# ORNL/HydraGNN

Measured on NVIDIA H100. Metric: atoms_per_sec_training_step, higher is better.
Workload: dtype tf32

## Files before the change

### hydragnn_b200/csrc/hgb_tc.cu

```cuda
#include "hgb_tc.cuh"

namespace {

__device__ __forceinline__ void wgmma_n32(float* d, uint64_t ad, uint64_t bd) {
  asm volatile(
      "{\n"
      ".reg .pred p;\n"
      "setp.ne.b32 p, %18, 0;\n"
      "wgmma.mma_async.sync.aligned.m64n32k8.f32.tf32.tf32 "
      "{%0, %1, %2, %3, %4, %5, %6, %7, %8, %9, %10, %11, %12, %13, %14, %15}, %16, %17, p, 1, 1;\n"
      "}"
      : "+f"(d[0]), "+f"(d[1]), "+f"(d[2]), "+f"(d[3]), "+f"(d[4]), "+f"(d[5]), "+f"(d[6]), "+f"(d[7]), "+f"(d[8]), "+f"(d[9]),
        "+f"(d[10]), "+f"(d[11]), "+f"(d[12]), "+f"(d[13]), "+f"(d[14]), "+f"(d[15])
      : "l"(ad), "l"(bd), "r"(1));
}
__device__ __forceinline__ void wgmma_n16(float* d, uint64_t ad, uint64_t bd) {
  asm volatile(
      "{\n"
      ".reg .pred p;\n"
      "setp.ne.b32 p, %10, 0;\n"
      "wgmma.mma_async.sync.aligned.m64n16k8.f32.tf32.tf32 "
      "{%0, %1, %2, %3, %4, %5, %6, %7}, %8, %9, p, 1, 1;\n"
      "}"
      : "+f"(d[0]), "+f"(d[1]), "+f"(d[2]), "+f"(d[3]), "+f"(d[4]), "+f"(d[5]), "+f"(d[6]), "+f"(d[7])
      : "l"(ad), "l"(bd), "r"(1));
}

__device__ __forceinline__ float tf32_rna(float x) { return __uint_as_float((__float_as_uint(x) + 0x1000u) & 0xffffe000u); }

__device__ __forceinline__ void split_f4(const float4 v, float4& h, float4& l) {
  h.x = tf32_rna(v.x); h.y = tf32_rna(v.y); h.z = tf32_rna(v.z); h.w = tf32_rna(v.w);
  l.x = tf32_rna(v.x - h.x); l.y = tf32_rna(v.y - h.y); l.z = tf32_rna(v.z - h.z); l.w = tf32_rna(v.w - h.w);
}

struct LinParams {
  int m, kr, no;
  const float* w;
  int64_t ldw;
  int trans_b;
  const float* bias;
  int act;
  float act_param;
  float* y;
  float* z;
  const float* addend;
  int64_t ldy;
  const float* gsrc;
  int gact;
  int z_deriv;
  int stages;
  int split;
  int slots;
};

struct LinParamsGA : LinParams {
  const float* gadd;
  const int32_t* gptr;
  int ng;
  int64_t ldg;
};
template <bool GA> struct LinParamsOf { using type = LinParams; };
template <> struct LinParamsOf<true> { using type = LinParamsGA; };

constexpr int TILE_M = 64;
constexpr uint32_t A_STAGE = TILE_M * 128;
constexpr uint32_t SUB_BYTES = TILE_M * 128;
constexpr int LIN_THREADS = 384;

enum { EPI_NONE, EPI_RELU, EPI_SILU, EPI_SILU_ZD, EPI_TANH, EPI_OTHER };

template <int K, bool GA>
__device__ __forceinline__ float lin_epilogue1(const LinParams& p, float v, float& z, float a, float g) {
  z = v;
  if (K == EPI_RELU) v = isnan(v) ? v : fmaxf(v, 0.f);
  if (K == EPI_SILU) v = __fdividef(v, 1.f + __expf(-v));
  if (K == EPI_SILU_ZD) {
    const float s = __fdividef(1.f, 1.f + __expf(-v));
    v *= s;
    z = fmaf(v, 1.f - s, s);
  }
  if (K == EPI_TANH) v = tanhf(v);
  if (K == EPI_OTHER) v = hgb_act(v, p.act, p.act_param);
  if (GA || p.addend) v += a;
  if (p.gsrc) {
    if (p.gact == HGB_ACT_RELU_SELECT) v = hgb_relu_select(v, g);
    else v *= p.gact == HGB_ACT_DERIV ? g : hgb_act_grad(g, g, p.gact, p.act_param);
  }
  return v;
}

template <int K, bool GA>
__device__ __forceinline__ void lin_epilogue_sub(const LinParams& p, const float* sb, uint8_t* ys, uint8_t* zs, int tid, const float4* a,
                                                 const float4* g) {
#pragma unroll
  for (int j = 0; j < 4; ++j) {
    const int idx = j * 128 + tid, r = idx >> 3, q = idx & 7;
    const uint32_t off = (uint32_t)r * 128 + ((q ^ (r & 7)) << 4);
    float4 v = *reinterpret_cast<float4*>(ys + off), z;
    v.x = lin_epilogue1<K, GA>(p, v.x + sb[4 * q], z.x, a[j].x, g[j].x);
    v.y = lin_epilogue1<K, GA>(p, v.y + sb[4 * q + 1], z.y, a[j].y, g[j].y);
    v.z = lin_epilogue1<K, GA>(p, v.z + sb[4 * q + 2], z.z, a[j].z, g[j].z);
    v.w = lin_epilogue1<K, GA>(p, v.w + sb[4 * q + 3], z.w, a[j].w, g[j].w);
    *reinterpret_cast<float4*>(ys + off) = v;
    if (zs) *reinterpret_cast<float4*>(zs + off) = z;
  }
}

__device__ __forceinline__ int lin_graph_of(const LinParamsGA& p, int row) {
  int lo = 0, hi = p.ng;
  while (hi - lo > 1) {
    const int mid = (lo + hi) >> 1;
    if (__ldg(p.gptr + mid) <= row) lo = mid; else hi = mid;
  }
  return lo;
}

template <bool GA>
__device__ __forceinline__ void lin_load_operands(const typename LinParamsOf<GA>::type& p, int row0, int c, int tid, const int* gid, float4* a, float4* g) {
#pragma unroll
  for (int j = 0; j < 4; ++j) {
    const int idx = j * 128 + tid, row = row0 + (idx >> 3);
    const int64_t o = (int64_t)row * p.ldy + c * 32 + (idx & 7) * 4;
    const bool in = row < p.m;
    if (p.addend) a[j] = in ? __ldg(reinterpret_cast<const float4*>(p.addend + o)) : make_float4(0.f, 0.f, 0.f, 0.f);
    if constexpr (GA)
      a[j] = in ? __ldg(reinterpret_cast<const float4*>(p.gadd + (int64_t)gid[j] * p.ldg + c * 32 + (idx & 7) * 4))
                : make_float4(0.f, 0.f, 0.f, 0.f);
    if (p.gsrc) g[j] = in ? __ldg(reinterpret_cast<const float4*>(p.gsrc + o)) : make_float4(0.f, 0.f, 0.f, 0.f);
  }
}

template <int NC, bool SPLIT, bool GA>
__global__ void __launch_bounds__(LIN_THREADS, 1) tc_linear_kernel(const __grid_constant__ CUtensorMap tmap_a,
                                                                   const __grid_constant__ CUtensorMap tmap_y,
                                                                   const __grid_constant__ CUtensorMap tmap_z,
                                                                   const typename LinParamsOf<GA>::type p) {
  constexpr int NO = NC * 32;
  extern __shared__ uint8_t smem_raw[];
  uint8_t* smem = reinterpret_cast<uint8_t*>((reinterpret_cast<uintptr_t>(smem_raw) + 1023) & ~(uintptr_t)1023);
  const int KB = p.kr >> 5;
  const uint32_t b_pad = ((uint32_t)KB * NO * 128 + 1023) & ~1023u;
  uint8_t* sB = smem;
  uint8_t* sBlo = sB + b_pad;
  uint8_t* sOut = sB + (SPLIT ? 2 : 1) * (size_t)b_pad;
  uint8_t* sA = sOut + (size_t)2 * p.slots * SUB_BYTES;
  const int S = p.stages;
  const int SR = S >> 1;
  uint8_t* sAlo = sA + (size_t)S * A_STAGE;
  uint64_t* full = reinterpret_cast<uint64_t*>(sA + (size_t)(SPLIT ? 2 : 1) * S * A_STAGE);
  uint64_t* empty = full + S;
  uint64_t* full2 = empty + S;
  float* sbias = reinterpret_cast<float*>(full2 + S);

  const int warp = threadIdx.x >> 5, lane = threadIdx.x & 31;
  const int ntiles = (p.m + TILE_M - 1) / TILE_M;
  for (int i = threadIdx.x; i < NO; i += blockDim.x) sbias[i] = p.bias ? __ldg(p.bias + i) : 0.f;
  if (threadIdx.x == 0) {
    for (int s = 0; s < S; ++s) { mbar_init(full + s, 1); mbar_init(empty + s, 4); mbar_init(full2 + s, 3); }
    fence_barrier_init();
  }
  __syncthreads();

  if (warp < 4) {
    regs_dec<PRODUCER_REGS>();
    if (warp == 0) {
    if (lane == 0) {
      uint32_t li = 0;
      for (int t = blockIdx.x; t < ntiles; t += gridDim.x, ++li)
        for (int kb = 0; kb < KB; ++kb) {
          const uint32_t n = (li >> 1) * KB + kb;
          const int s = (li & 1) * SR + n % SR;
          mbar_wait(empty + s, ((n / SR) & 1) ^ 1);
          mbar_expect_tx(full + s, A_STAGE);
          tma_load_2d(sA + (size_t)s * A_STAGE, &tmap_a, full + s, kb * 32, t * TILE_M);
        }
    }
    } else {
    if (SPLIT) {
      const int tl = threadIdx.x - 32;
      uint32_t li = 0;
      for (int t = blockIdx.x; t < ntiles; t += gridDim.x, ++li)
        for (int kb = 0; kb < KB; ++kb) {
          const uint32_t n = (li >> 1) * KB + kb;
          const int s = (li & 1) * SR + n % SR;
          mbar_wait(full + s, (n / SR) & 1);
          float4* pa = reinterpret_cast<float4*>(sA + (size_t)s * A_STAGE);
          float4* pl = reinterpret_cast<float4*>(sAlo + (size_t)s * A_STAGE);
          for (int idx = tl; idx < (int)(A_STAGE / 16); idx += 96) {
            float4 h, l;
            split_f4(pa[idx], h, l);
            pa[idx] = h;
            pl[idx] = l;
          }
          fence_proxy_async();
          __syncwarp();
          if (lane == 0) mbar_arrive(full2 + s);
        }
    }
    }
  } else {
    regs_inc<CONSUMER_REGS>();
    {
      const int total = NO * p.kr;
      constexpr int SU = 8;
      for (int base = threadIdx.x - 128; base < total; base += 256 * SU) {
        float val[SU];
        uint32_t off[SU];
#pragma unroll
        for (int u = 0; u < SU; ++u) {
          const int i = base + u * 256;
          val[u] = 0.f;
          off[u] = 0xffffffffu;
          if (i < total) {
            if (!p.trans_b) {
              const int r = i / p.kr, c = i - r * p.kr;
              off[u] = kmajor_sw128_off(r, c, NO);
              val[u] = __ldg(p.w + (int64_t)r * p.ldw + c);
            } else {
              const int c = i / NO, r = i - c * NO;
              off[u] = kmajor_sw128_off(r, c, NO);
              val[u] = __ldg(p.w + (int64_t)c * p.ldw + r);
            }
          }
        }
#pragma unroll
        for (int u = 0; u < SU; ++u)
          if (off[u] != 0xffffffffu) {
            if (SPLIT) {
              const float hi = tf32_rna(val[u]);
              *reinterpret_cast<float*>(sB + off[u]) = hi;
              *reinterpret_cast<float*>(sBlo + off[u]) = tf32_rna(val[u] - hi);
            } else {
              *reinterpret_cast<float*>(sB + off[u]) = val[u];
            }
          }
      }
      fence_proxy_async();
    }
    named_bar_sync(1, 256);
    const int cw = (warp - 4) >> 2;
    const int wq = warp & 3;
    const int tid = threadIdx.x & 127;
    const uint32_t sA_addr = smem_u32(sA), sAlo_addr = smem_u32(sAlo), sB_addr = smem_u32(sB), sBlo_addr = smem_u32(sBlo);
    uint8_t* sOwn = sOut + (size_t)cw * p.slots * SUB_BYTES;
    const int per_sub = p.z ? 2 : 1;
    const int ahead = p.slots / per_sub - 1;
    const int kind = p.act == HGB_ACT_NONE ? EPI_NONE
                     : p.act == HGB_ACT_RELU ? EPI_RELU
                     : p.act == HGB_ACT_SILU ? (p.z && p.z_deriv ? EPI_SILU_ZD : EPI_SILU)
                     : p.act == HGB_ACT_TANH ? EPI_TANH
                                             : EPI_OTHER;
    const bool operands = GA || p.addend || p.gsrc;
    float acc[NC * 16];
    uint32_t sub = 0;
    int li = cw;
    for (int t = blockIdx.x + cw * gridDim.x; t < ntiles; t += 2 * gridDim.x, li += 2) {
      const int row0 = t * TILE_M;
      int gid[4] = {0, 0, 0, 0};
      if constexpr (GA) {
#pragma unroll
        for (int j = 0; j < 4; ++j) {
          const int row = row0 + ((j * 128 + tid) >> 3);
          if (row < p.m) gid[j] = lin_graph_of(p, row);
        }
      }
      float4 opa[4], opg[4];
#pragma unroll
      for (int j = 0; j < 4; ++j) opa[j] = opg[j] = make_float4(0.f, 0.f, 0.f, 0.f);
      constexpr bool early = NC < 8;
      if (early && operands) lin_load_operands<GA>(p, row0, 0, tid, gid, opa, opg);
#pragma unroll
      for (int j = 0; j < NC * 16; ++j) acc[j] = 0.f;
      const uint32_t n0 = (uint32_t)(li >> 1) * KB;
      for (int kb = 0; kb < KB; ++kb) {
        const uint32_t n = n0 + kb;
        const int s = cw * SR + n % SR;
        mbar_wait(SPLIT ? full2 + s : full + s, (n / SR) & 1);
        fence_regs<NC * 16>(acc);
        wgmma_fence();
#pragma unroll
        for (int k4 = 0; k4 < 4; ++k4) {
          const uint64_t ad = make_desc(sA_addr + s * A_STAGE + k4 * 32);
          const uint32_t boff = (uint32_t)kb * NO * 128 + k4 * 32;
          const uint64_t bd = make_desc(sB_addr + boff);
          if (SPLIT) {
            wgmma_tf32<NC>(acc, make_desc(sAlo_addr + s * A_STAGE + k4 * 32), bd);
            wgmma_tf32<NC>(acc, ad, make_desc(sBlo_addr + boff));
          }
          wgmma_tf32<NC>(acc, ad, bd);
        }
        wgmma_commit();
        fence_regs<NC * 16>(acc);
        if (kb > 0) {
          wgmma_wait<1>();
          if (lane == 0) mbar_arrive(empty + cw * SR + (n - 1) % SR);
        }
      }
      wgmma_wait<0>();
      fence_regs<NC * 16>(acc);
      if (lane == 0) mbar_arrive(empty + cw * SR + (n0 + KB - 1) % SR);
      if (!early && operands) lin_load_operands<GA>(p, row0, 0, tid, gid, opa, opg);
#pragma unroll 1
      for (int c = 0; c < NC; ++c, ++sub) {
        uint8_t* ys = sOwn + (size_t)((sub % (p.slots / per_sub)) * per_sub) * SUB_BYTES;
        uint8_t* zs = p.z ? ys + SUB_BYTES : nullptr;
        if (tid == 0) {
          if (ahead == 0) bulk_wait_read<0>(); else if (ahead == 1) bulk_wait_read<1>(); else bulk_wait_read<3>();
        }
        named_bar_sync(2 + cw, 128);
#pragma unroll
        for (int cc = 0; cc < NC; ++cc)
          if (cc == c) {
#pragma unroll
            for (int i = 0; i < 4; ++i)
#pragma unroll
              for (int h = 0; h < 2; ++h) {
                const int r = wq * 16 + (lane >> 2) + 8 * h, col = i * 8 + 2 * (lane & 3);
                *reinterpret_cast<float2*>(ys + kmajor_sw128_off(r, col, TILE_M)) =
                    make_float2(acc[16 * cc + 4 * i + 2 * h], acc[16 * cc + 4 * i + 2 * h + 1]);
              }
          }
        named_bar_sync(2 + cw, 128);
        const float* sb = sbias + c * 32;
        switch (kind) {
          case EPI_NONE: lin_epilogue_sub<EPI_NONE, GA>(p, sb, ys, zs, tid, opa, opg); break;
          case EPI_RELU: lin_epilogue_sub<EPI_RELU, GA>(p, sb, ys, zs, tid, opa, opg); break;
          case EPI_SILU: lin_epilogue_sub<EPI_SILU, GA>(p, sb, ys, zs, tid, opa, opg); break;
          case EPI_SILU_ZD: lin_epilogue_sub<EPI_SILU_ZD, GA>(p, sb, ys, zs, tid, opa, opg); break;
          case EPI_TANH: lin_epilogue_sub<EPI_TANH, GA>(p, sb, ys, zs, tid, opa, opg); break;
          default: lin_epilogue_sub<EPI_OTHER, GA>(p, sb, ys, zs, tid, opa, opg);
        }
        if (operands && c + 1 < NC) lin_load_operands<GA>(p, row0, c + 1, tid, gid, opa, opg);
        fence_proxy_async();
        named_bar_sync(2 + cw, 128);
        if (tid == 0) {
          tma_store_2d(&tmap_y, ys, c * 32, row0);
          if (zs) tma_store_2d(&tmap_z, zs, c * 32, row0);
          bulk_commit();
        }
      }
    }
    if (tid == 0) bulk_wait_all();
  }
}

struct WgParams {
  int m, no, ko;
  int chunks_per_cta;
  int stages;
  int tbufs;
  int split;
  int flush;
  float* part;
};

constexpr int WG_ROWS = 32;
constexpr int WG_NA = 128;
constexpr int WG_THREADS = 384;

template <int Q, bool SPLIT>
__global__ void __launch_bounds__(WG_THREADS, 1) tc_wgrad_kernel(const __grid_constant__ CUtensorMap tmap_dz,
                                                                 const __grid_constant__ CUtensorMap tmap_x, const WgParams p) {
  constexpr int KO = 32 * Q, NB = KO + 16;
  constexpr uint32_t SLAB = WG_ROWS * 128;
  constexpr uint32_t HI_BYTES = (uint32_t)(WG_NA + NB) * 128;
  extern __shared__ uint8_t smem_raw[];
  uint8_t* smem = reinterpret_cast<uint8_t*>((reinterpret_cast<uintptr_t>(smem_raw) + 1023) & ~(uintptr_t)1023);
  const int n0 = blockIdx.y * WG_NA;
  const int nrows = min(WG_NA, p.no - n0);
  const int nsl = nrows >> 5;
  const uint32_t raw_bytes = (uint32_t)(nsl + Q) * SLAB;
  const uint32_t tb_bytes = HI_BYTES * (SPLIT ? 2 : 1);
  const int S = p.stages, T = p.tbufs;
  uint8_t* tbuf = smem;
  uint8_t* raw = smem + (size_t)T * tb_bytes;
  uint64_t* full = reinterpret_cast<uint64_t*>(raw + (size_t)S * raw_bytes);
  uint64_t* empty = full + S;
  const int warp = threadIdx.x >> 5, lane = threadIdx.x & 31;

  const int total_chunks = (p.m + WG_ROWS - 1) / WG_ROWS;
  const int c_beg = blockIdx.x * p.chunks_per_cta;
  const int nchunks = max(0, min(total_chunks, c_beg + p.chunks_per_cta) - c_beg);

  if (threadIdx.x == 0) {
    for (int s = 0; s < S; ++s) { mbar_init(full + s, 1); mbar_init(empty + s, 8); }
    fence_barrier_init();
  }
  for (int i = threadIdx.x; i < (int)(T * tb_bytes / 4); i += blockDim.x) {
    const uint32_t o = (uint32_t)i * 4 % tb_bytes;
    const bool lo = o >= HI_BYTES;
    const int row = (int)((lo ? o - HI_BYTES : o) / 128);
    reinterpret_cast<float*>(tbuf)[i] = (!lo && row >= WG_NA + KO) ? 1.f : 0.f;
  }
  fence_proxy_async();
  __syncthreads();

  if (warp >= 8) {
    regs_dec<PRODUCER_REGS>();
    if (warp == 8 && lane == 0) {
      for (int c = 0; c < nchunks; ++c) {
        const int s = c % S;
        mbar_wait(empty + s, ((c / S) & 1) ^ 1);
        mbar_expect_tx(full + s, raw_bytes);
        uint8_t* st = raw + (size_t)s * raw_bytes;
        const int row0 = (c_beg + c) * WG_ROWS;
        for (int j = 0; j < nsl; ++j) tma_load_2d(st + (size_t)j * SLAB, &tmap_dz, full + s, n0 + j * 32, row0);
        for (int j = 0; j < Q; ++j) tma_load_2d(st + (size_t)(nsl + j) * SLAB, &tmap_x, full + s, j * 32, row0);
      }
    }
    return;
  }

  regs_inc<CONSUMER_REGS>();
  const int wg = warp >> 2, wq = warp & 3;
  const bool mma_on = wg * 64 < nrows;
  const int rows_t = nsl * 32 + KO;
  float acc[Q][16], accb[8];
#pragma unroll
  for (int c = 0; c < Q; ++c)
#pragma unroll
    for (int j = 0; j < 16; ++j) acc[c][j] = 0.f;
#pragma unroll
  for (int j = 0; j < 8; ++j) accb[j] = 0.f;
  bool first = true;
  float* part = p.part + (size_t)blockIdx.x * p.no * (p.ko + 1);

  auto flush = [&]() {
    if (mma_on) {
      const int rb = n0 + wg * 64 + wq * 16 + (lane >> 2);
#pragma unroll
      for (int h = 0; h < 2; ++h) {
        const int row = rb + 8 * h;
        if (row < n0 + nrows) {
          float* pr = part + (size_t)row * (KO + 1);
#pragma unroll
          for (int c = 0; c < Q; ++c)
#pragma unroll
            for (int i = 0; i < 4; ++i)
#pragma unroll
              for (int e = 0; e < 2; ++e) {
                const int col = c * 32 + i * 8 + 2 * (lane & 3) + e;
                const float v = acc[c][4 * i + 2 * h + e];
                pr[col] = first ? v : pr[col] + v;
              }
          if ((lane & 3) == 0) pr[KO] = first ? accb[2 * h] : pr[KO] + accb[2 * h];
        }
      }
    }
    first = false;
#pragma unroll
    for (int c = 0; c < Q; ++c)
#pragma unroll
      for (int j = 0; j < 16; ++j) acc[c][j] = 0.f;
#pragma unroll
    for (int j = 0; j < 8; ++j) accb[j] = 0.f;
  };

  for (int c = 0; c < nchunks; ++c) {
    const int s = c % S;
    uint8_t* tb = tbuf + (size_t)(c % T) * tb_bytes;
    const uint8_t* st = raw + (size_t)s * raw_bytes;
    mbar_wait(full + s, (c / S) & 1);
    for (int it = threadIdx.x; it < rows_t * 8; it += 256) {
      const int r = it % rows_t, m4 = it / rows_t;
      const int slab = r < nrows ? r >> 5 : nsl + ((r - nrows) >> 5);
      const float* src = reinterpret_cast<const float*>(st + (size_t)slab * SLAB) + (r & 31) + m4 * 4 * 32;
      const float4 v = make_float4(src[0], src[32], src[64], src[96]);
      const int orow = r < nrows ? r : WG_NA + (r - nrows);
      const uint32_t off = (uint32_t)orow * 128 + ((m4 ^ (orow & 7)) << 4);
      if (SPLIT) {
        float4 h, l;
        split_f4(v, h, l);
        *reinterpret_cast<float4*>(tb + off) = h;
        *reinterpret_cast<float4*>(tb + HI_BYTES + off) = l;
      } else {
        *reinterpret_cast<float4*>(tb + off) = v;
      }
    }
    fence_proxy_async();
    __syncwarp();
    if (lane == 0) mbar_arrive(empty + s);
    named_bar_sync(1, 256);
    if (mma_on) {
      const uint32_t ta = smem_u32(tb);
      fence_regs<Q * 16>(&acc[0][0]);
      fence_regs<8>(accb);
      wgmma_fence();
#pragma unroll
      for (int k4 = 0; k4 < 4; ++k4) {
        const uint32_t aoff = (uint32_t)(wg * 64) * 128 + k4 * 32;
        const uint64_t ad = make_desc(ta + aoff), adl = make_desc(ta + HI_BYTES + aoff);
#pragma unroll
        for (int j = 0; j < Q; ++j) {
          const uint32_t boff = (uint32_t)WG_NA * 128 + (uint32_t)j * 4096 + k4 * 32;
          const uint64_t bd = make_desc(ta + boff);
          if (SPLIT) {
            wgmma_n32(acc[j], adl, bd);
            wgmma_n32(acc[j], ad, make_desc(ta + HI_BYTES + boff));
          }
          wgmma_n32(acc[j], ad, bd);
        }
        const uint64_t bones = make_desc(ta + (uint32_t)(WG_NA + KO) * 128 + k4 * 32);
        if (SPLIT) wgmma_n16(accb, adl, bones);
        wgmma_n16(accb, ad, bones);
      }
      wgmma_commit();
      fence_regs<Q * 16>(&acc[0][0]);
      fence_regs<8>(accb);
    }
    if (T == 2) wgmma_wait<1>(); else wgmma_wait<0>();
    if (p.flush && (c + 1) % p.flush == 0 && c + 1 < nchunks) {
      wgmma_wait<0>();
      fence_regs<Q * 16>(&acc[0][0]);
      fence_regs<8>(accb);
      flush();
    }
    named_bar_sync(2, 256);
  }
  wgmma_wait<0>();
  fence_regs<Q * 16>(&acc[0][0]);
  fence_regs<8>(accb);
  flush();
}

__global__ void tc_wgrad_reduce_kernel(const float* __restrict__ part, int nparts, int no, int ko, float* __restrict__ dw,
                                       int64_t lddw, float* __restrict__ db, int accumulate) {
  __shared__ float red[8][33];
  const int w = ko + 1;
  const int cnt = no * w;
  const int i = blockIdx.x * 32 + threadIdx.x;
  float acc = 0.f;
  if (i < cnt) {
    float a0 = 0.f, a1 = 0.f, a2 = 0.f, a3 = 0.f;
    int b = threadIdx.y;
    for (; b + 24 < nparts; b += 32) {
      a0 += part[(size_t)b * cnt + i]; a1 += part[(size_t)(b + 8) * cnt + i];
      a2 += part[(size_t)(b + 16) * cnt + i]; a3 += part[(size_t)(b + 24) * cnt + i];
    }
    for (; b < nparts; b += 8) a0 += part[(size_t)b * cnt + i];
    acc = (a0 + a1) + (a2 + a3);
  }
  red[threadIdx.y][threadIdx.x] = acc;
  __syncthreads();
  if (threadIdx.y == 0 && i < cnt) {
    float t = 0.f;
#pragma unroll
    for (int w8 = 0; w8 < 8; ++w8) t += red[w8][threadIdx.x];
    const int r = i / w, c = i % w;
    if (c == ko) {
      if (db) db[r] = accumulate ? db[r] + t : t;
    } else {
      float* o = dw + (int64_t)r * lddw + c;
      *o = accumulate ? *o + t : t;
    }
  }
}

bool shape_ok(int kr, int no) { return kr >= 32 && kr <= 256 && kr % 32 == 0 && no >= 32 && no <= 256 && no % 32 == 0; }

template <int NC, bool SPLIT, bool GA>
void launch_linear_t(int grid, size_t smem, cudaStream_t st, const CUtensorMap* tm, const typename LinParamsOf<GA>::type& p) {
  static bool attr_set = false;
  if (!attr_set) {
    cudaFuncSetAttribute(tc_linear_kernel<NC, SPLIT, GA>, cudaFuncAttributeMaxDynamicSharedMemorySize, (int)SMEM_MAX);
    attr_set = true;
  }
  tc_linear_kernel<NC, SPLIT, GA><<<grid, LIN_THREADS, smem, st>>>(tm[0], tm[1], tm[2], p);
}
template <int NC>
void launch_linear(int grid, size_t smem, cudaStream_t st, const CUtensorMap* tm, const LinParamsGA& p) {
  if (p.gadd) {
    if (p.split) launch_linear_t<NC, true, true>(grid, smem, st, tm, p); else launch_linear_t<NC, false, true>(grid, smem, st, tm, p);
  } else {
    const LinParams& q = p;
    if (q.split) launch_linear_t<NC, true, false>(grid, smem, st, tm, q); else launch_linear_t<NC, false, false>(grid, smem, st, tm, q);
  }
}

template <int Q, bool SPLIT>
void launch_wgrad_t(dim3 grid, size_t smem, cudaStream_t st, const CUtensorMap& tdz, const CUtensorMap& tx, const WgParams& p) {
  static bool attr_set = false;
  if (!attr_set) {
    cudaFuncSetAttribute(tc_wgrad_kernel<Q, SPLIT>, cudaFuncAttributeMaxDynamicSharedMemorySize, (int)SMEM_MAX);
    attr_set = true;
  }
  tc_wgrad_kernel<Q, SPLIT><<<grid, WG_THREADS, smem, st>>>(tdz, tx, p);
}
template <int Q>
void launch_wgrad(dim3 grid, size_t smem, cudaStream_t st, const CUtensorMap& tdz, const CUtensorMap& tx, const WgParams& p) {
  if (p.split) launch_wgrad_t<Q, true>(grid, smem, st, tdz, tx, p); else launch_wgrad_t<Q, false>(grid, smem, st, tdz, tx, p);
}

}

static bool wide_ok(int kr, int no) { return kr >= 32 && kr <= 1024 && kr % 32 == 0 && no >= 32 && no <= 1024 && no % 32 == 0; }

extern "C" int hgb_tc_linear_supported(int32_t m, int32_t n_out, int32_t k_red) { return (m >= 128 && wide_ok(k_red, n_out)) ? 1 : 0; }

static int tc_linear_piece(const float* a, int64_t lda, const float* w, int64_t ldw, int32_t trans_b, const float* bias, int32_t m,
                           int32_t n_out, int32_t k_red, int32_t act, float act_param, float* y, float* z, const float* addend,
                           const float* gsrc, int32_t gact, int64_t ldy, int32_t exact, const float* gadd, int64_t ldg,
                           const int32_t* gptr, int32_t ng, hgb_stream_t stream) {
  HGB_REQUIRE(a && w && y && m >= 128 && shape_ok(k_red, n_out), "tc_linear: unsupported shape m=%d n=%d k=%d", m, n_out, k_red);
  HGB_REQUIRE(lda % 4 == 0 && ldy % 4 == 0 && ((uintptr_t)a % 16 == 0) && ((uintptr_t)y % 16 == 0) && (!z || (uintptr_t)z % 16 == 0) &&
                  (!addend || (uintptr_t)addend % 16 == 0) && (!gsrc || (uintptr_t)gsrc % 16 == 0) &&
                  (!gadd || ((uintptr_t)gadd % 16 == 0 && ldg % 4 == 0)),
              "tc_linear: operands must be 16-byte aligned with a row stride that is a multiple of 4");
  CUtensorMap tm[3];
  int rc = make_tmap(&tm[0], a, m, k_red, lda, TILE_M, CU_TENSOR_MAP_SWIZZLE_128B);
  if (rc) return rc;
  LinParamsGA p;
  p.m = m; p.kr = k_red; p.no = n_out; p.w = w; p.ldw = ldw; p.trans_b = trans_b; p.bias = bias; p.act = act; p.act_param = act_param;
  p.y = y; p.z = z; p.addend = addend; p.ldy = ldy; p.gsrc = gsrc; p.gact = gact; p.z_deriv = (!gsrc && gact == HGB_ACT_DERIV) ? 1 : 0;
  p.gadd = gadd; p.gptr = gptr; p.ng = ng; p.ldg = ldg;
  rc = make_tmap(&tm[1], y, m, n_out, ldy, TILE_M, CU_TENSOR_MAP_SWIZZLE_128B);
  if (rc) return rc;
  rc = make_tmap(&tm[2], z ? z : y, m, n_out, ldy, TILE_M, CU_TENSOR_MAP_SWIZZLE_128B);
  if (rc) return rc;
  const int KB = k_red / 32;
  const int dup = exact ? 2 : 1;
  const size_t b_bytes = ((size_t)KB * n_out * 128 + 1023) & ~(size_t)1023;
  int stages = 0, slots = 0;
  size_t fixed = 0;
  for (slots = 4; slots >= 2; slots -= 2) {
    fixed = 1024 + dup * b_bytes + (size_t)2 * slots * SUB_BYTES + (size_t)n_out * 4 + 64;
    stages = fixed < SMEM_MAX ? (int)((SMEM_MAX - fixed) / (dup * A_STAGE + 3 * 8)) : 0;
    if (stages > 8) stages = 8;
    stages &= ~1;
    if (stages >= 4) break;
  }
  HGB_REQUIRE(stages >= 4, "tc_linear: weight operand does not fit shared memory (n=%d k=%d)", n_out, k_red);
  p.stages = stages;
  p.slots = slots;
  p.split = exact ? 1 : 0;
  const size_t smem = fixed + (size_t)stages * (dup * A_STAGE + 3 * 8);
  const int ntiles = (m + TILE_M - 1) / TILE_M;
  const int grid = ntiles < HGB_NUM_SMS ? ntiles : HGB_NUM_SMS;
  cudaStream_t st = (cudaStream_t)stream;
  switch (n_out / 32) {
    case 1: launch_linear<1>(grid, smem, st, tm, p); break;
    case 2: launch_linear<2>(grid, smem, st, tm, p); break;
    case 3: launch_linear<3>(grid, smem, st, tm, p); break;
    case 4: launch_linear<4>(grid, smem, st, tm, p); break;
    case 5: launch_linear<5>(grid, smem, st, tm, p); break;
    case 6: launch_linear<6>(grid, smem, st, tm, p); break;
    case 7: launch_linear<7>(grid, smem, st, tm, p); break;
    default: launch_linear<8>(grid, smem, st, tm, p); break;
  }
  HGB_LAUNCH_CHECK("tc_linear");
  return HGB_OK;
}

static int tc_linear_pieces(const float* a, int64_t lda, const float* w, int64_t ldw, int32_t trans_b, const float* bias, int32_t m,
                            int32_t n_out, int32_t k_red, int32_t act, float act_param, float* y, float* z, const float* addend,
                            const float* gsrc, int32_t gact, int32_t exact, const float* gadd, int64_t ldg, const int32_t* gptr, int32_t ng,
                            hgb_stream_t stream) {
  HGB_REQUIRE(a && w && y && hgb_tc_linear_supported(m, n_out, k_red), "tc_linear: unsupported shape m=%d n=%d k=%d", m, n_out, k_red);
  HGB_REQUIRE(k_red <= 256 || (act == HGB_ACT_NONE && !z && !gsrc), "tc_linear: reduction length %d > 256 needs a plain linear layer", k_red);
  const int kc_max = k_red < 256 ? k_red : 256;
  int nc_max = (int)(((exact ? 64 : 160) * 1024) / (4 * (size_t)kc_max) / 32) * 32;
  if (nc_max > 256) nc_max = 256;
  for (int c0 = 0; c0 < n_out; c0 += nc_max) {
    const int nc = n_out - c0 < nc_max ? n_out - c0 : nc_max;
    for (int k0 = 0; k0 < k_red; k0 += 256) {
      const int kc = k_red - k0 < 256 ? k_red - k0 : 256;
      const float* wp = trans_b ? w + (int64_t)k0 * ldw + c0 : w + (int64_t)c0 * ldw + k0;
      const float* add = k0 == 0 ? (addend ? addend + c0 : nullptr) : y + c0;
      int rc = tc_linear_piece(a + k0, lda, wp, ldw, trans_b, (bias && k0 == 0) ? bias + c0 : nullptr, m, nc, kc, act, act_param, y + c0,
                               z ? z + c0 : nullptr, add, gsrc ? gsrc + c0 : nullptr, gact, n_out, exact,
                               (gadd && k0 == 0) ? gadd + c0 : nullptr, ldg, gptr, ng, stream);
      if (rc) return rc;
    }
  }
  return HGB_OK;
}

extern "C" int hgb_tc_linear(const float* a, int64_t lda, const float* w, int64_t ldw, int32_t trans_b, const float* bias, int32_t m,
                             int32_t n_out, int32_t k_red, int32_t act, float act_param, float* y, float* z, const float* addend,
                             const float* gsrc, int32_t gact, int32_t exact, hgb_stream_t stream) {
  return tc_linear_pieces(a, lda, w, ldw, trans_b, bias, m, n_out, k_red, act, act_param, y, z, addend, gsrc, gact, exact, nullptr, 0,
                          nullptr, 0, stream);
}

extern "C" int hgb_tc_linear_graph_add(const float* a, int64_t lda, const float* w, int64_t ldw, int32_t m, int32_t n_out, int32_t k_red,
                                       const float* gadd, int64_t ldg, const int32_t* gptr, int32_t ng, float* y, int32_t exact,
                                       hgb_stream_t stream) {
  HGB_REQUIRE(a && w && y && gadd && gptr && ng >= 1 && hgb_tc_linear_supported(m, n_out, k_red),
              "tc_linear_graph_add: unsupported shape m=%d n=%d k=%d graphs=%d", m, n_out, k_red, ng);
  return tc_linear_pieces(a, lda, w, ldw, 0, nullptr, m, n_out, k_red, HGB_ACT_NONE, 0.f, y, nullptr, nullptr, nullptr, 0, exact, gadd, ldg,
                          gptr, ng, stream);
}

extern "C" int64_t hgb_tc_wgrad_workspace_bytes(int32_t n_out, int32_t k_out) { return (int64_t)HGB_NUM_SMS * n_out * (k_out + 1) * 4; }

extern "C" int hgb_tc_wgrad(const float* dz, int64_t lddz, const float* x, int64_t ldx, int32_t m, int32_t n_out, int32_t k_out,
                            float* dw, int64_t lddw, float* db, int32_t accumulate, int32_t exact, void* workspace,
                            int64_t workspace_bytes, hgb_stream_t stream) {
  HGB_REQUIRE(dz && x && dw && workspace && m >= 128 && shape_ok(k_out, n_out) && k_out + 16 <= 256,
              "tc_wgrad: unsupported shape m=%d n=%d k=%d", m, n_out, k_out);
  HGB_REQUIRE(lddz % 4 == 0 && ldx % 4 == 0 && ((uintptr_t)dz % 16 == 0) && ((uintptr_t)x % 16 == 0), "tc_wgrad: operands must be 16-byte aligned");
  HGB_REQUIRE(workspace_bytes >= hgb_tc_wgrad_workspace_bytes(n_out, k_out), "tc_wgrad: workspace too small");
  WgParams p;
  p.m = m; p.no = n_out; p.ko = k_out;
  p.split = exact ? 1 : 0;
  p.flush = exact ? 8 : 0;
  const int Q = k_out / 32;
  const int nsl_max = (n_out < WG_NA ? n_out : WG_NA) / 32;
  const size_t raw_bytes = (size_t)(nsl_max + Q) * WG_ROWS * 128;
  const size_t tb_bytes = (size_t)(WG_NA + k_out + 16) * 128 * (exact ? 2 : 1);
  const size_t budget = SMEM_MAX - 1024 - 256;
  int tbufs = 2;
  int stages = budget > 2 * tb_bytes ? (int)((budget - 2 * tb_bytes) / raw_bytes) : 0;
  if (stages < 2) {
    tbufs = 1;
    stages = (int)((budget - tb_bytes) / raw_bytes);
  }
  if (stages > 4) stages = 4;
  HGB_REQUIRE(stages >= 2, "tc_wgrad: stage does not fit shared memory");
  p.stages = stages;
  p.tbufs = tbufs;
  CUtensorMap tdz, tx;
  int rc = make_tmap(&tdz, dz, m, n_out, lddz, WG_ROWS, CU_TENSOR_MAP_SWIZZLE_NONE);
  if (rc) return rc;
  rc = make_tmap(&tx, x, m, k_out, ldx, WG_ROWS, CU_TENSOR_MAP_SWIZZLE_NONE);
  if (rc) return rc;
  const int total_chunks = (m + WG_ROWS - 1) / WG_ROWS;
  const int gy = (n_out + WG_NA - 1) / WG_NA;
  const int max_x = HGB_NUM_SMS / gy;
  int gx = total_chunks < max_x ? total_chunks : max_x;
  p.chunks_per_cta = (total_chunks + gx - 1) / gx;
  gx = (total_chunks + p.chunks_per_cta - 1) / p.chunks_per_cta;
  p.part = (float*)workspace;
  const size_t smem = 1024 + tbufs * tb_bytes + stages * raw_bytes + 2 * stages * 8;
  cudaStream_t st = (cudaStream_t)stream;
  const dim3 grid(gx, gy);
  switch (Q) {
    case 1: launch_wgrad<1>(grid, smem, st, tdz, tx, p); break;
    case 2: launch_wgrad<2>(grid, smem, st, tdz, tx, p); break;
    case 3: launch_wgrad<3>(grid, smem, st, tdz, tx, p); break;
    case 4: launch_wgrad<4>(grid, smem, st, tdz, tx, p); break;
    case 5: launch_wgrad<5>(grid, smem, st, tdz, tx, p); break;
    case 6: launch_wgrad<6>(grid, smem, st, tdz, tx, p); break;
    default: launch_wgrad<7>(grid, smem, st, tdz, tx, p); break;
  }
  HGB_LAUNCH_CHECK("tc_wgrad");
  const int outs = n_out * (k_out + 1);
  tc_wgrad_reduce_kernel<<<(outs + 31) / 32, dim3(32, 8), 0, st>>>(p.part, gx, n_out, k_out, dw, lddw, db, accumulate);
  HGB_LAUNCH_CHECK("tc_wgrad_reduce");
  return HGB_OK;
}
```

Before: 44.31 million.

## Split wgrad kernel into dedicated transposer warps pipelined with MMA warpgroups

```diff
diff --git a/hydragnn_b200/csrc/hgb_tc.cu b/hydragnn_b200/csrc/hgb_tc.cu
--- a/hydragnn_b200/csrc/hgb_tc.cu
+++ b/hydragnn_b200/csrc/hgb_tc.cu
@@ -356,7 +356,9 @@
 
 constexpr int WG_ROWS = 32;
 constexpr int WG_NA = 128;
-constexpr int WG_THREADS = 384;
+constexpr int WG_TRANSPOSERS = 7;
+constexpr int WG_THREADS = 256 + 32 * (1 + WG_TRANSPOSERS);
+constexpr int WG_AUX_REGS = 40, WG_MMA_REGS = 216;
 
 template <int Q, bool SPLIT>
 __global__ void __launch_bounds__(WG_THREADS, 1) tc_wgrad_kernel(const __grid_constant__ CUtensorMap tmap_dz,
@@ -369,6 +371,7 @@
   const int n0 = blockIdx.y * WG_NA;
   const int nrows = min(WG_NA, p.no - n0);
   const int nsl = nrows >> 5;
+  const int n_mma_wg = (nrows + 63) >> 6;
   const uint32_t raw_bytes = (uint32_t)(nsl + Q) * SLAB;
   const uint32_t tb_bytes = HI_BYTES * (SPLIT ? 2 : 1);
   const int S = p.stages, T = p.tbufs;
@@ -376,6 +379,8 @@
   uint8_t* raw = smem + (size_t)T * tb_bytes;
   uint64_t* full = reinterpret_cast<uint64_t*>(raw + (size_t)S * raw_bytes);
   uint64_t* empty = full + S;
+  uint64_t* tfull = empty + S;
+  uint64_t* tempty = tfull + T;
   const int warp = threadIdx.x >> 5, lane = threadIdx.x & 31;
 
   const int total_chunks = (p.m + WG_ROWS - 1) / WG_ROWS;
@@ -383,106 +388,116 @@
   const int nchunks = max(0, min(total_chunks, c_beg + p.chunks_per_cta) - c_beg);
 
   if (threadIdx.x == 0) {
-    for (int s = 0; s < S; ++s) { mbar_init(full + s, 1); mbar_init(empty + s, 8); }
+    for (int s = 0; s < S; ++s) { mbar_init(full + s, 1); mbar_init(empty + s, WG_TRANSPOSERS); }
+    for (int t = 0; t < T; ++t) { mbar_init(tfull + t, WG_TRANSPOSERS); mbar_init(tempty + t, 4 * n_mma_wg); }
     fence_barrier_init();
   }
-  for (int i = threadIdx.x; i < (int)(T * tb_bytes / 4); i += blockDim.x) {
-    const uint32_t o = (uint32_t)i * 4 % tb_bytes;
-    const bool lo = o >= HI_BYTES;
-    const int row = (int)((lo ? o - HI_BYTES : o) / 128);
-    reinterpret_cast<float*>(tbuf)[i] = (!lo && row >= WG_NA + KO) ? 1.f : 0.f;
+  {
+    const int zrows = WG_NA - nrows, frows = zrows + 16;
+    const int words = T * (SPLIT ? 2 : 1) * frows * 32;
+    for (int i = threadIdx.x; i < words; i += blockDim.x) {
+      const int rr = (i >> 5) % frows, half = (i >> 5) / frows;
+      const int row = rr < zrows ? nrows + rr : WG_NA + KO + (rr - zrows);
+      const bool lo = SPLIT && (half & 1);
+      const int t = SPLIT ? half >> 1 : half;
+      reinterpret_cast<float*>(tbuf + (size_t)t * tb_bytes + (lo ? HI_BYTES : 0) + (size_t)row * 128)[i & 31] =
+          (!lo && rr >= zrows) ? 1.f : 0.f;
+    }
   }
   fence_proxy_async();
   __syncthreads();
 
   if (warp >= 8) {
-    regs_dec<PRODUCER_REGS>();
-    if (warp == 8 && lane == 0) {
-      for (int c = 0; c < nchunks; ++c) {
-        const int s = c % S;
-        mbar_wait(empty + s, ((c / S) & 1) ^ 1);
-        mbar_expect_tx(full + s, raw_bytes);
-        uint8_t* st = raw + (size_t)s * raw_bytes;
-        const int row0 = (c_beg + c) * WG_ROWS;
-        for (int j = 0; j < nsl; ++j) tma_load_2d(st + (size_t)j * SLAB, &tmap_dz, full + s, n0 + j * 32, row0);
-        for (int j = 0; j < Q; ++j) tma_load_2d(st + (size_t)(nsl + j) * SLAB, &tmap_x, full + s, j * 32, row0);
+    regs_dec<WG_AUX_REGS>();
+    if (warp == 8) {
+      if (lane == 0) {
+        for (int c = 0; c < nchunks; ++c) {
+          const int s = c % S;
+          mbar_wait(empty + s, ((c / S) & 1) ^ 1);
+          mbar_expect_tx(full + s, raw_bytes);
+          uint8_t* st = raw + (size_t)s * raw_bytes;
+          const int row0 = (c_beg + c) * WG_ROWS;
+          for (int j = 0; j < nsl; ++j) tma_load_2d(st + (size_t)j * SLAB, &tmap_dz, full + s, n0 + j * 32, row0);
+          for (int j = 0; j < Q; ++j) tma_load_2d(st + (size_t)(nsl + j) * SLAB, &tmap_x, full + s, j * 32, row0);
+        }
+      }
+      return;
+    }
+    const int tw = warp - 9;
+    const int units = (nsl + Q) * 8;
+    for (int c = 0; c < nchunks; ++c) {
+      const int s = c % S, t = c % T;
+      uint8_t* tb = tbuf + (size_t)t * tb_bytes;
+      const uint8_t* st = raw + (size_t)s * raw_bytes;
+      mbar_wait(full + s, (c / S) & 1);
+      mbar_wait(tempty + t, ((c / T) & 1) ^ 1);
+#pragma unroll 4
+      for (int u = tw; u < units; u += WG_TRANSPOSERS) {
+        const int slab = u >> 3, m4 = u & 7;
+        const float* src = reinterpret_cast<const float*>(st + (size_t)slab * SLAB) + lane + m4 * 4 * 32;
+        const float4 v = make_float4(src[0], src[32], src[64], src[96]);
+        const int orow = slab < nsl ? slab * 32 + lane : WG_NA + (slab - nsl) * 32 + lane;
+        const uint32_t off = (uint32_t)orow * 128 + ((m4 ^ (orow & 7)) << 4);
+        if (SPLIT) {
+          float4 h, l;
+          split_f4(v, h, l);
+          *reinterpret_cast<float4*>(tb + off) = h;
+          *reinterpret_cast<float4*>(tb + HI_BYTES + off) = l;
+        } else {
+          *reinterpret_cast<float4*>(tb + off) = v;
+        }
+      }
+      fence_proxy_async();
+      __syncwarp();
+      if (lane == 0) {
+        mbar_arrive(empty + s);
+        mbar_arrive(tfull + t);
       }
     }
     return;
   }
 
-  regs_inc<CONSUMER_REGS>();
+  regs_inc<WG_MMA_REGS>();
   const int wg = warp >> 2, wq = warp & 3;
-  const bool mma_on = wg * 64 < nrows;
-  const int rows_t = nsl * 32 + KO;
+  if (wg >= n_mma_wg) return;
   float acc[Q][16], accb[8];
-#pragma unroll
-  for (int c = 0; c < Q; ++c)
-#pragma unroll
-    for (int j = 0; j < 16; ++j) acc[c][j] = 0.f;
-#pragma unroll
-  for (int j = 0; j < 8; ++j) accb[j] = 0.f;
-  bool first = true;
   float* part = p.part + (size_t)blockIdx.x * p.no * (p.ko + 1);
 
-  auto flush = [&]() {
-    if (mma_on) {
-      const int rb = n0 + wg * 64 + wq * 16 + (lane >> 2);
-#pragma unroll
-      for (int h = 0; h < 2; ++h) {
-        const int row = rb + 8 * h;
-        if (row < n0 + nrows) {
-          float* pr = part + (size_t)row * (KO + 1);
-#pragma unroll
-          for (int c = 0; c < Q; ++c)
-#pragma unroll
-            for (int i = 0; i < 4; ++i)
-#pragma unroll
-              for (int e = 0; e < 2; ++e) {
-                const int col = c * 32 + i * 8 + 2 * (lane & 3) + e;
-                const float v = acc[c][4 * i + 2 * h + e];
-                pr[col] = first ? v : pr[col] + v;
-              }
-          if ((lane & 3) == 0) pr[KO] = first ? accb[2 * h] : pr[KO] + accb[2 * h];
-        }
-      }
-    }
-    first = false;
-#pragma unroll
-    for (int c = 0; c < Q; ++c)
-#pragma unroll
-      for (int j = 0; j < 16; ++j) acc[c][j] = 0.f;
+  auto store = [&](bool first) {
+    const int rb = n0 + wg * 64 + wq * 16 + (lane >> 2);
+#pragma unroll
+    for (int h = 0; h < 2; ++h) {
+      const int row = rb + 8 * h;
+      if (row < n0 + nrows) {
+        float* pr = part + (size_t)row * (KO + 1);
+#pragma unroll
+        for (int c = 0; c < Q; ++c)
+#pragma unroll
+          for (int i = 0; i < 4; ++i)
+#pragma unroll
+            for (int e = 0; e < 2; ++e) {
+              const int col = c * 32 + i * 8 + 2 * (lane & 3) + e;
+              const float v = acc[c][4 * i + 2 * h + e];
+              pr[col] = first ? v : pr[col] + v;
+            }
+        if ((lane & 3) == 0) pr[KO] = first ? accb[2 * h] : pr[KO] + accb[2 * h];
+      }
+    }
+  };
+
+  int c = 0;
+  for (bool first = true;; first = false) {
+#pragma unroll
+    for (int q = 0; q < Q; ++q)
+#pragma unroll
+      for (int j = 0; j < 16; ++j) acc[q][j] = 0.f;
 #pragma unroll
     for (int j = 0; j < 8; ++j) accb[j] = 0.f;
-  };
-
-  for (int c = 0; c < nchunks; ++c) {
-    const int s = c % S;
-    uint8_t* tb = tbuf + (size_t)(c % T) * tb_bytes;
-    const uint8_t* st = raw + (size_t)s * raw_bytes;
-    mbar_wait(full + s, (c / S) & 1);
-    for (int it = threadIdx.x; it < rows_t * 8; it += 256) {
-      const int r = it % rows_t, m4 = it / rows_t;
-      const int slab = r < nrows ? r >> 5 : nsl + ((r - nrows) >> 5);
-      const float* src = reinterpret_cast<const float*>(st + (size_t)slab * SLAB) + (r & 31) + m4 * 4 * 32;
-      const float4 v = make_float4(src[0], src[32], src[64], src[96]);
-      const int orow = r < nrows ? r : WG_NA + (r - nrows);
-      const uint32_t off = (uint32_t)orow * 128 + ((m4 ^ (orow & 7)) << 4);
-      if (SPLIT) {
-        float4 h, l;
-        split_f4(v, h, l);
-        *reinterpret_cast<float4*>(tb + off) = h;
-        *reinterpret_cast<float4*>(tb + HI_BYTES + off) = l;
-      } else {
-        *reinterpret_cast<float4*>(tb + off) = v;
-      }
-    }
-    fence_proxy_async();
-    __syncwarp();
-    if (lane == 0) mbar_arrive(empty + s);
-    named_bar_sync(1, 256);
-    if (mma_on) {
-      const uint32_t ta = smem_u32(tb);
+    const int c_end = p.flush ? min(nchunks, c + p.flush) : nchunks;
+    for (; c < c_end; ++c) {
+      const int t = c % T;
+      const uint32_t ta = smem_u32(tbuf + (size_t)t * tb_bytes);
+      mbar_wait(tfull + t, (c / T) & 1);
       fence_regs<Q * 16>(&acc[0][0]);
       fence_regs<8>(accb);
       wgmma_fence();
@@ -507,20 +522,20 @@
       wgmma_commit();
       fence_regs<Q * 16>(&acc[0][0]);
       fence_regs<8>(accb);
-    }
-    if (T == 2) wgmma_wait<1>(); else wgmma_wait<0>();
-    if (p.flush && (c + 1) % p.flush == 0 && c + 1 < nchunks) {
-      wgmma_wait<0>();
-      fence_regs<Q * 16>(&acc[0][0]);
-      fence_regs<8>(accb);
-      flush();
-    }
-    named_bar_sync(2, 256);
-  }
-  wgmma_wait<0>();
-  fence_regs<Q * 16>(&acc[0][0]);
-  fence_regs<8>(accb);
-  flush();
+      if (T >= 2) {
+        wgmma_wait<1>();
+        if (c > 0 && lane == 0) mbar_arrive(tempty + (c - 1) % T);
+      } else {
+        wgmma_wait<0>();
+        if (lane == 0) mbar_arrive(tempty + t);
+      }
+    }
+    wgmma_wait<0>();
+    fence_regs<Q * 16>(&acc[0][0]);
+    fence_regs<8>(accb);
+    store(first);
+    if (c >= nchunks) break;
+  }
 }
 
 __global__ void tc_wgrad_reduce_kernel(const float* __restrict__ part, int nparts, int no, int ko, float* __restrict__ dw,
@@ -708,14 +723,11 @@
   const int nsl_max = (n_out < WG_NA ? n_out : WG_NA) / 32;
   const size_t raw_bytes = (size_t)(nsl_max + Q) * WG_ROWS * 128;
   const size_t tb_bytes = (size_t)(WG_NA + k_out + 16) * 128 * (exact ? 2 : 1);
-  const size_t budget = SMEM_MAX - 1024 - 256;
-  int tbufs = 2;
-  int stages = budget > 2 * tb_bytes ? (int)((budget - 2 * tb_bytes) / raw_bytes) : 0;
-  if (stages < 2) {
-    tbufs = 1;
-    stages = (int)((budget - tb_bytes) / raw_bytes);
-  }
-  if (stages > 4) stages = 4;
+  const size_t budget = SMEM_MAX - 1024;
+  int tbufs = 3;
+  while (tbufs > 1 && (size_t)tbufs * (tb_bytes + 16) + 2 * (raw_bytes + 16) > budget) --tbufs;
+  const size_t left = budget > (size_t)tbufs * (tb_bytes + 16) ? budget - (size_t)tbufs * (tb_bytes + 16) : 0;
+  const int stages = (int)(left / (raw_bytes + 16));
   HGB_REQUIRE(stages >= 2, "tc_wgrad: stage does not fit shared memory");
   p.stages = stages;
   p.tbufs = tbufs;
@@ -731,7 +743,7 @@
   p.chunks_per_cta = (total_chunks + gx - 1) / gx;
   gx = (total_chunks + p.chunks_per_cta - 1) / p.chunks_per_cta;
   p.part = (float*)workspace;
-  const size_t smem = 1024 + tbufs * tb_bytes + stages * raw_bytes + 2 * stages * 8;
+  const size_t smem = 1024 + tbufs * (tb_bytes + 16) + stages * (raw_bytes + 16);
   cudaStream_t st = (cudaStream_t)stream;
   const dim3 grid(gx, gy);
   switch (Q) {
diff --git a/profiles/wgrad_bench.py b/profiles/wgrad_bench.py
--- /dev/null
+++ b/profiles/wgrad_bench.py
@@ -0,0 +1,144 @@
+import argparse
+import json
+import os
+import subprocess
+import sys
+
+sys.path.insert(0, os.path.dirname(os.path.dirname(os.path.abspath(__file__))))
+import torch
+import hydragnn_b200 as hb
+from hydragnn_b200 import _lib, ops
+from hydragnn_b200.synthetic import ARCH, WORKLOADS, make_samples
+
+GRAPHS = {"qm9_painn": 16384, "md17_egnn": 8192, "lj_egnn": 4096}
+dev = torch.device("cuda")
+
+
+def card():
+    q = subprocess.run(["nvidia-smi", "--query-gpu=name,power.limit", "--format=csv,noheader", "-i", str(torch.cuda.current_device())],
+                       capture_output=True, text=True)
+    return q.stdout.strip() if q.returncode == 0 else torch.cuda.get_device_name()
+
+
+def traced_wgrad_calls(name, precision):
+    G = GRAPHS[name]
+    w = WORKLOADS[name]
+    b = make_samples(name, G).to(dev)
+    b._num_graphs = G
+    pbc = w.get("pbc") or w.get("pbc_box")
+    b = (hb.get_radius_graph_pbc if pbc else hb.get_radius_graph)(w["radius"], w["max_neighbours"])(b)
+    kw = dict(ARCH[name])
+    mlip = bool(kw.get("enable_interatomic_potential"))
+    model = hb.get_distributed_model(hb.set_precision(hb.create_model(**kw), precision))
+    opt = hb.FlatAdamW(model, lr=1e-3)
+    hi = None if mlip else hb.get_head_indices(model, b)
+    hb.train_step(model, opt, b, compute_grad_energy=mlip, head_index=hi)
+    torch.cuda.synchronize()
+    _lib.trace_begin()
+    hb.train_step(model, opt, b, compute_grad_energy=mlip, head_index=hi)
+    torch.cuda.synchronize()
+    calls = _lib.trace_end()
+    del model, opt, b
+    torch.cuda.empty_cache()
+    return [(a["m"], a["n_out"], a["k_out"], a["lddz"], a["ldx"], a["exact"]) for e, a, _ in calls if e == "hgb_tc_wgrad"]
+
+
+class Call:
+
+    def __init__(self, m, n_out, k_out, lddz, ldx, exact):
+        g = torch.Generator(device=dev).manual_seed(0)
+        self.dz = torch.randn(m, lddz, device=dev, generator=g)
+        self.x = torch.randn(m, ldx, device=dev, generator=g)
+        self.dw = torch.empty(n_out, k_out, device=dev)
+        self.db = torch.empty(n_out, device=dev)
+        self.nbytes = _lib.query("hgb_tc_wgrad_workspace_bytes", n_out, k_out)
+        self.ws = torch.empty(self.nbytes, dtype=torch.uint8, device=dev)
+        self.args = (m, n_out, k_out, lddz, ldx, exact)
+
+    def __call__(self):
+        m, n_out, k_out, lddz, ldx, exact = self.args
+        _lib.call("hgb_tc_wgrad", self.dz.data_ptr(), lddz, self.x.data_ptr(), ldx, m, n_out, k_out, self.dw.data_ptr(), k_out,
+                  self.db.data_ptr(), 0, exact, self.ws.data_ptr(), self.nbytes, torch.cuda.current_stream().cuda_stream)
+
+
+def time_warm(fn, iters):
+    for _ in range(3):
+        fn()
+    a, b = torch.cuda.Event(enable_timing=True), torch.cuda.Event(enable_timing=True)
+    a.record()
+    for _ in range(iters):
+        fn()
+    b.record()
+    torch.cuda.synchronize()
+    return a.elapsed_time(b) / iters * 1e3
+
+
+def time_cold(fn, iters, flush):
+    ts = []
+    for it in range(iters + 3):
+        flush.zero_()
+        a, b = torch.cuda.Event(enable_timing=True), torch.cuda.Event(enable_timing=True)
+        a.record()
+        fn()
+        b.record()
+        torch.cuda.synchronize()
+        if it >= 3:
+            ts.append(a.elapsed_time(b) * 1e3)
+    return sum(ts) / len(ts)
+
+
+def fit(xs, ys):
+    n = len(xs)
+    mx, my = sum(xs) / n, sum(ys) / n
+    sxx = sum((x - mx) ** 2 for x in xs)
+    slope = sum((x - mx) * (y - my) for x, y in zip(xs, ys)) / sxx
+    return slope, my - slope * mx
+
+
+def main():
+    ap = argparse.ArgumentParser()
+    ap.add_argument("--workloads", default="qm9_painn:bf16,lj_egnn:fp32,md17_egnn:fp32")
+    ap.add_argument("--iters", type=int, default=40)
+    a = ap.parse_args()
+    torch.cuda.set_device(0)
+    flush = torch.empty(256 * 1024 * 1024, dtype=torch.uint8, device=dev)
+    print(json.dumps({"card": card(), "library": _lib.LIB_PATH}), flush=True)
+    for spec in a.workloads.split(","):
+        name, precision = spec.split(":")
+        calls = traced_wgrad_calls(name, precision)
+        shapes = {}
+        for c in calls:
+            shapes[c] = shapes.get(c, 0) + 1
+        tot = {"warm": 0.0, "cold": 0.0}
+        tot_bytes = 0
+        for (m, n_out, k_out, lddz, ldx, exact), count in shapes.items():
+            row = {"workload": name, "m": m, "n_out": n_out, "k_out": k_out, "lddz": lddz, "ldx": ldx, "mode": "exact" if exact else "tf32",
+                   "calls_per_step": count}
+            for kind in ("warm", "cold"):
+                xs, ys = [], []
+                for f in (0.25, 0.5, 1.0, 2.0):
+                    mm = max(128, int(m * f))
+                    call = Call(mm, n_out, k_out, lddz, ldx, exact)
+                    t = time_warm(call, a.iters) if kind == "warm" else time_cold(call, a.iters, flush)
+                    alg = mm * (n_out + k_out) * 4
+                    xs.append(alg)
+                    ys.append(t)
+                    if f == 1.0:
+                        row["%s_us_at_m" % kind] = round(t, 2)
+                        row["%s_GBps_at_m" % kind] = round(alg / t * 1e-3, 1)
+                        tot[kind] += t * count
+                        if kind == "warm":
+                            tot_bytes += alg * count
+                    del call
+                slope, icpt = fit(xs, ys)
+                row["%s_stream_GBps" % kind] = round(1e-3 / slope, 1)
+                row["%s_fixed_us" % kind] = round(icpt, 2)
+            print(json.dumps(row), flush=True)
+        print(json.dumps({"workload": name, "total_calls_per_step": len(calls), "alg_GB": round(tot_bytes / 1e9, 3),
+                          "warm_us": round(tot["warm"], 1), "cold_us": round(tot["cold"], 1),
+                          "warm_GBps": round(tot_bytes / tot["warm"] * 1e-3, 1), "cold_GBps": round(tot_bytes / tot["cold"] * 1e-3, 1),
+                          "card": card()}), flush=True)
+
+
+if __name__ == "__main__":
+    main()
```

New measurement: 46.38 million, median of 6. +4.7%, better.
